# ucla-mobility/QuantV2X

Hardware: AMD Instinct MI355X
Metric: frames/sec/node (N-agent int8 BEV fusion) (higher is better)
Workload: dtype i8

## Files before the change

### include/qv2x.h

```cpp
#ifndef QV2X_H
#define QV2X_H

#include <stdint.h>

#ifdef __cplusplus
extern "C" {
#endif
#if defined(__GNUC__) || defined(__clang__)
#pragma GCC visibility push(default)
#endif

#define QV2X_OK 0
#define QV2X_EINVAL (-1)
#define QV2X_EALIGN (-2)
#define QV2X_MAX_GROUPS 4

const char* qv2x_last_error(void);
#define QV2X_ABI_VERSION 9
int qv2x_version(void);

int qv2x_fill_i8(int8_t* buf, int64_t bytes, int value, void* stream);

int64_t qv2x_voxelize_workspace_bytes(int n_points);
int qv2x_voxelize_f32(const float* points, int n_points, const float* lidar_range, const float* voxel_size, int agent,
// ... 57 lines not shown
                   int8_t* out, void* stream);

int qv2x_deconv_i8_batch(const qv2x_deconv_desc* descs , int n, const int8_t* const* ins ,
                         const float* const* ws, const float* const* biases, int8_t* const* outs, void* stream);

typedef struct {
    int32_t n, h, w;
    int32_t levels, kc;
    int32_t in_zx;
    float in_delta;
    int32_t segs;
} qv2x_encode_desc;
int64_t qv2x_codebook_level_floats(int kc);
int qv2x_codebook_c2_f32(const float* codebook, int kc, float* c2, void* stream);
int qv2x_codebook_encode_f32(const qv2x_encode_desc* desc , const int8_t* in,
                             const float* const* level_weights ,
                             uint8_t* codes, void* stream);
int qv2x_codebook_encode_wave_f32(const qv2x_encode_desc* desc , const int8_t* in, const float* in_f32,
                                  const float* const* level_weights , uint8_t* codes, void* stream);

int qv2x_codebook_encode_collapsed_f32(const qv2x_encode_desc* desc , const int8_t* in, const float* g_packed, const float* bias,
                                       const float* tables, uint8_t* codes, void* stream);

int qv2x_codebook_encode_candidates_i8(const qv2x_encode_desc* desc , const int8_t* in, const int8_t* g_limbs, const double* bias_packed,
                                       const int32_t* tables, const float* tau , uint8_t* codes, uint32_t* list, uint32_t* counters,
                                       void* stream);
int qv2x_codebook_encode_listed_f32(const qv2x_encode_desc* desc , const int8_t* in, const float* const* level_weights ,
                                    const uint32_t* list, const uint32_t* list_count, uint8_t* codes, void* stream);

int qv2x_codebook_encode_candidates_seg_i8(const qv2x_encode_desc* desc , const int8_t* in, const int8_t* g_limbs, const double* bias_packed,
                                           const int32_t* tables, const float* tau , uint8_t* codes, uint32_t* list, uint32_t* counters,
                                           void* stream);

typedef struct {
    int32_t agents, h, w, levels, kc;
    int32_t max_cav, ego;
    int64_t code_agent_stride, code_level_stride;
    double h_metres, w_metres, discrete_ratio;
    int32_t fusion;
} qv2x_fuse_desc;
int qv2x_fuse_att_f32(const qv2x_fuse_desc* desc , const uint8_t* codes, const float* lut, const float* lut_bias,
                      const float* feats, const double* pairwise, float* fused, void* stream);

int qv2x_fuse_att_batch_f32(const qv2x_fuse_desc* desc , int n_scenes, const int64_t* scene_offset ,
                            const int32_t* scene_agents , const uint8_t* codes, const float* lut, const float* lut_bias,
                            const float* feats, const double* pairwise, float* fused, void* stream);

int qv2x_decode_lut_f32(const uint8_t* codes, int R, int levels, int kc, const float* lut, const float* lut_bias,
                        float* out, void* stream);

int qv2x_dequant_i8_f32(const int8_t* in, int n, int h, int w, int c, int zp, float delta, float* out, void* stream);
// ... 188 lines not shown
```

### quantv2x_amd/csrc/codebook_encode.h

```cpp
#pragma once
#include "common.h"

namespace qv2x {

constexpr int ENC_D = 256;
constexpr int ENC_WAVE_PAD = 16 * 256;

struct EncArgs {
    const int8_t* in; const float* in_f32; uint8_t* codes;
    const float* lvl[4];
    int n, h, w, levels, kc, ax, M;
    int segs, ke;
    float dx;
    int m_lo, m_hi;
    int list_slots = 1, list_tail_max = 0;
    const unsigned* list = nullptr; const unsigned* list_count = nullptr;
};

__device__ __host__ __forceinline__ int64_t level_floats_wg(int kc) { return 3LL * (ENC_D * ENC_D + ENC_D) + (int64_t)ENC_D * kc + (int64_t)kc * ENC_D + kc; }
__device__ __host__ __forceinline__ int64_t level_floats(int kc) { return level_floats_wg(kc) + 3LL * ENC_D * ENC_D + (int64_t)((kc + 63) / 64 * 64) * ENC_D + ENC_WAVE_PAD; }

struct ListPlan { int n[3], first[3], total, full; };
__device__ __forceinline__ ListPlan list_plan(const EncArgs& a) {
    ListPlan p;
    int t = 0;
#pragma unroll
    for (int c = 0; c < 3; ++c) { p.n[c] = (int)a.list_count[1 + c]; p.first[c] = t; t += (p.n[c] + 31) >> 5; }
    p.total = t;
    const int full = t / a.list_slots * a.list_slots;
    p.full = t - full > a.list_tail_max ? t : full;
    return p;
}
__device__ __forceinline__ void list_tile(const ListPlan& p, int tile, int& cls, int& i0) {
    cls = tile >= p.first[2] ? 2 : (tile >= p.first[1] ? 1 : 0);
    i0 = (tile - p.first[cls]) * 32;
}

int encode_wave_launch(const EncArgs& a, hipStream_t st);
int encode_wave_list_launch(const EncArgs& a, int waves, hipStream_t st);

}
```

### quantv2x_amd/csrc/codebook_encode.hip

```cpp
#include <cstdlib>

#include <atomic>

#include "codebook_encode.h"

namespace qv2x {

#ifdef QV2X_ENC_TRACE
__device__ unsigned long long g_enc_blk[4096][4];
#endif
#ifdef QV2X_ENC_FINE
__device__ long long g_enc_fine[2048][40];
#define EFINE(k) do { if (threadIdx.x == 0 && blockIdx.x < 2048) g_enc_fine[blockIdx.x][12 * l + (k)] = __builtin_amdgcn_s_memtime(); } while (0)
#else
#define EFINE(k) do { } while (0)
#endif

constexpr int LDF = 258;
__device__ __forceinline__ int kpos(int c) { return (c & ~3) | ((c & 1) << 1) | ((c >> 1) & 1); }
constexpr int D = 256;
#ifndef QV2X_ENC_LDS_PAD
#define QV2X_ENC_LDS_PAD 0
#endif

// ... 304 lines not shown
                for (int r = 0; r < 16; ++r) bufA[(i * 32 + mfma32_row(r, lane)) * LDF + kpos(col)] = acc[i][r] - cv[i][r];
            lds_barrier();
            EFINE(11);
        }
    }
#ifdef QV2X_ENC_TRACE
    if (tid == 0 && blockIdx.x < 4096) {
        g_enc_blk[blockIdx.x][0] = t_start; g_enc_blk[blockIdx.x][1] = __builtin_readcyclecounter();
        g_enc_blk[blockIdx.x][2] = hwid; g_enc_blk[blockIdx.x][3] = xcc;
    }
#endif
}

template <int ER, bool EXT = false>
__global__ __launch_bounds__(512, ER == 32 ? 4 : 2) void codebook_encode_kernel(const EncArgs a) {
    __shared__ __attribute__((aligned(16))) float smem[enc_smem_floats<ER>()];
    encode_rows<ER, EXT>(a, a.m_lo + blockIdx.x * ER, smem);
}

template <bool EXT>
__global__ __launch_bounds__(512, 2) void codebook_encode_list_tail_kernel(const EncArgs a) {
    __shared__ __attribute__((aligned(16))) float smem[enc_smem_floats<32>()];
    const ListPlan plan = list_plan(a);
    for (int t = plan.full + (int)blockIdx.x; t < plan.total; t += (int)gridDim.x) {
        int cls, i0;
        list_tile(plan, t, cls, i0);
        encode_rows<32, EXT, true>(a, i0, smem, a.list + (size_t)cls * a.M, plan.n[cls], cls);
        __syncthreads();
    }
}

template <bool EXT>
__global__ __launch_bounds__(512, 2) void codebook_encode_mixed_kernel(const EncArgs a, const int n64) {
    __shared__ __attribute__((aligned(16))) float smem[enc_smem_floats<64>()];
    if ((int)blockIdx.x < n64) encode_rows<64, EXT>(a, a.m_lo + blockIdx.x * 64, smem);
    else encode_rows<32, EXT>(a, a.m_lo + n64 * 64 + ((int)blockIdx.x - n64) * 32, smem);
}

__global__ void codebook_c2_kernel(const float* __restrict__ cb, int kc, float* __restrict__ c2) {
    const int k = blockIdx.x * blockDim.x + threadIdx.x;
    if (k >= kc) return;
    float s[4];
    for (int q = 0; q < 4; ++q) {
        float acc = 0.0f;
        for (int i = 0; i < 64; ++i) { const float v = cb[(size_t)k * D + q * 64 + i]; acc = fmaf(v, v, acc); }
        s[q] = acc;
    }
// ... 11 lines not shown

extern "C" int64_t qv2x_codebook_level_floats(int kc) { return qv2x::level_floats(kc); }

static int encode_launch(const qv2x_encode_desc* d, const int8_t* in, const float* in_f32, const float* const* level_weights, uint8_t* codes, void* stream,
                         int form = 0);

extern "C" int qv2x_codebook_encode_wave_f32(const qv2x_encode_desc* d, const int8_t* in, const float* in_f32, const float* const* level_weights,
                                             uint8_t* codes, void* stream) {
    if (!in && !in_f32) return qv2x::fail(QV2X_EINVAL, "qv2x_codebook_encode_wave_f32: null pointer");
    return encode_launch(d, in_f32 ? (const int8_t*)in_f32 : in, in_f32, level_weights, codes, stream, 1);
}

extern "C" int qv2x_codebook_encode_f32(const qv2x_encode_desc* d, const int8_t* in, const float* const* level_weights,
                                        uint8_t* codes, void* stream) {
    return encode_launch(d, in, nullptr, level_weights, codes, stream);
}

extern "C" int qv2x_codebook_encode_f32in(const qv2x_encode_desc* d, const float* in, const float* const* level_weights,
                                          uint8_t* codes, void* stream) {
    if (!in) return qv2x::fail(QV2X_EINVAL, "qv2x_codebook_encode_f32in: null pointer");
    return encode_launch(d, (const int8_t*)in, in, level_weights, codes, stream);
}

extern "C" int qv2x_codebook_encode_listed_f32(const qv2x_encode_desc* d, const int8_t* in, const float* const* level_weights,
                                               const uint32_t* list, const uint32_t* list_count, uint8_t* codes, void* stream) {
    using namespace qv2x;
    if (!d || !in || !level_weights || !codes || !list || !list_count) return fail(QV2X_EINVAL, "qv2x_codebook_encode_listed_f32: null pointer");
    if (d->n <= 0 || d->h <= 0 || d->w <= 0 || d->levels < 1 || d->levels > 4) return fail(QV2X_EINVAL, "qv2x_codebook_encode_listed_f32: bad shape");
    const int segs = d->segs ? d->segs : 1;
    if (segs != 1 && segs != 2) return fail(QV2X_EINVAL, "qv2x_codebook_encode_listed_f32: seg_num 1 or 2 (got %d)", d->segs);
    if (d->kc < 32 || d->kc > 256 || d->kc % 32 || (segs > 1 && d->kc % 64) || segs * d->kc > 32 * ENC_MAX_TILES)
        return fail(QV2X_EINVAL, "qv2x_codebook_encode_listed_f32: dict_size must be a multiple of 32 up to 256 (of 64 with two segments): got %d x %d", segs, d->kc);
    if ((uintptr_t)in & 15) return fail(QV2X_EALIGN, "qv2x_codebook_encode_listed_f32: in must be 16-byte aligned");
    EncArgs a;
    a.in = in; a.in_f32 = nullptr; a.codes = codes; a.n = d->n; a.h = d->h; a.w = d->w; a.levels = d->levels; a.kc = d->kc;
    a.segs = segs; a.ke = segs * d->kc;
    const bool ext = segs > 1 || a.ke > 128;
    a.ax = 128 - d->in_zx; a.dx = d->in_delta; a.M = d->n * d->h * d->w; a.m_lo = 0; a.m_hi = a.M;
    a.list = list; a.list_count = list_count;
    for (int l = 0; l < 4; ++l) {
        a.lvl[l] = l < d->levels ? level_weights[l] : nullptr;
        if (l < d->levels && (!a.lvl[l] || ((uintptr_t)a.lvl[l] & 15))) return fail(QV2X_EALIGN, "qv2x_codebook_encode_listed_f32: level %d weights null or unaligned", l);
    }
    int cus = 256, dev = 0, v = 0;
    if (hipGetDevice(&dev) == hipSuccess && hipDeviceGetAttribute(&v, hipDeviceAttributeMultiprocessorCount, dev) == hipSuccess && v > 0) cus = v;
    const int tiles = (a.M + 31) / 32;
    int tail_knob = 0;
#ifdef QV2X_DEV_KNOBS
    static const int tail_env = getenv("QV2X_LIST_TAIL") ? atoi(getenv("QV2X_LIST_TAIL")) : 0;
    tail_knob = tail_env;
#endif
    a.list_slots = 4 * cus; a.list_tail_max = tail_knob > 0 ? tail_knob : 2 * cus;
    const int grid_tail = 2 * cus;
    if (tiles + 3 >= 2 * a.list_slots) {
        if (int rc = encode_wave_list_launch(a, a.list_slots, (hipStream_t)stream)) return rc;
    } else {
        a.list_slots = 1 << 30; a.list_tail_max = 1 << 30;
    }
    if (ext) codebook_encode_list_tail_kernel<true><<<tiles < grid_tail ? tiles : grid_tail, 512, 0, (hipStream_t)stream>>>(a);
    else codebook_encode_list_tail_kernel<false><<<tiles < grid_tail ? tiles : grid_tail, 512, 0, (hipStream_t)stream>>>(a);
    return hip_check(hipGetLastError(), "qv2x_codebook_encode_listed_f32 launch");
}

static int encode_launch(const qv2x_encode_desc* d, const int8_t* in, const float* in_f32, const float* const* level_weights, uint8_t* codes, void* stream,
                         int form) {
    using namespace qv2x;
    if (!d || !in || !level_weights || !codes) return fail(QV2X_EINVAL, "qv2x_codebook_encode_f32: null pointer");
    if (d->n <= 0 || d->h <= 0 || d->w <= 0 || d->levels < 1 || d->levels > 4) return fail(QV2X_EINVAL, "qv2x_codebook_encode_f32: bad shape");
    const int segs = d->segs ? d->segs : 1;
    if (segs != 1 && segs != 2 && segs != 4) return fail(QV2X_EINVAL, "qv2x_codebook_encode_f32: seg_num must be 1, 2 or 4 (got %d)", d->segs);
    if (d->kc < 32 || d->kc > 256 || d->kc % 32 || (segs > 1 && d->kc % 64) || segs * d->kc > 32 * ENC_MAX_TILES)
        return fail(QV2X_EINVAL, "qv2x_codebook_encode_f32: dict_size must be a multiple of 32 up to 256 (of 64 with seg_num > 1; seg_num * dict_size <= %d): "
                                 "got dict_size %d, seg_num %d", 32 * ENC_MAX_TILES, d->kc, segs);
    if ((uintptr_t)in & 15) return fail(QV2X_EALIGN, "qv2x_codebook_encode_f32: in must be 16-byte aligned");
    EncArgs a;
    a.in = in; a.in_f32 = in_f32; a.codes = codes; a.n = d->n; a.h = d->h; a.w = d->w; a.levels = d->levels; a.kc = d->kc;
    a.segs = segs; a.ke = segs * d->kc;
    const bool ext = segs > 1 || a.ke > 128;
    a.ax = 128 - d->in_zx; a.dx = d->in_delta; a.M = d->n * d->h * d->w; a.m_lo = 0; a.m_hi = a.M;
    for (int l = 0; l < 4; ++l) {
        a.lvl[l] = l < d->levels ? level_weights[l] : nullptr;
// ... 63 lines not shown
```

### quantv2x_amd/csrc/codebook_encode_cand.hip

```cpp
#include "common.h"

namespace qv2x {
namespace {

struct CandArgs {
    const int8_t* in; const int8_t* gpack; const double* bias; const int* tables;
    uint8_t* codes; unsigned* list; unsigned* counters;
    float tau[3][3];
    int n, h, w, hw, M, levels, kc, ke, zx, gbytes, tbytes;
    float delta;
};

constexpr int NPF = 8;
constexpr int LIMBS = 3;
template <int V> struct IC { static constexpr int value = V; };

__device__ __forceinline__ double shfl_xor_f64(double v, int m) {
    const long long b = __builtin_bit_cast(long long, v);
    const int lo = __shfl_xor((int)b, m), hi = __shfl_xor((int)(b >> 32), m);
    return __builtin_bit_cast(double, ((long long)hi << 32) | (unsigned)lo);
}

template <int CT, int SEGS, int PACK>
__global__ __launch_bounds__(256) __attribute__((amdgpu_waves_per_eu(1, 1))) void encode_candidates_kernel(const CandArgs a) {
// ... 151 lines not shown
        const unsigned tot = wcnt[0][threadIdx.x] + wcnt[1][threadIdx.x] + wcnt[2][threadIdx.x] + wcnt[3][threadIdx.x];
        wbase[threadIdx.x] = tot ? atomicAdd(a.counters + 1 + threadIdx.x, tot) : 0u;
        if (tot) atomicAdd(a.counters, tot);
    }
    __syncthreads();
    unsigned base[3];
#pragma unroll
    for (int c = 0; c < 3; ++c) {
        base[c] = wbase[c];
        for (int w2 = 0; w2 < wave; ++w2) base[c] += wcnt[w2][c];
    }
#pragma unroll
    for (int c = 0; c < 3; ++c) {
        unsigned at = __builtin_amdgcn_readfirstlane(base[c]);
#pragma unroll
        for (int ct = 0; ct < CT; ++ct) {
            if (first[ct] == c && hf == 0 && m[ct] < a.M)
                a.list[(size_t)c * a.M + at + (unsigned)__builtin_popcountll(mask[c][ct] & ((1ull << lane) - 1ull))] = (unsigned)m[ct];
            at += (unsigned)__builtin_popcountll(mask[c][ct]);
        }
    }
}

__global__ void zero_counters_kernel(unsigned* c) { if (threadIdx.x < 4) c[threadIdx.x] = 0; }

template <int CT, int SEGS, int PACK>
void launch(const CandArgs& a, hipStream_t st) {
    encode_candidates_kernel<CT, SEGS, PACK><<<(a.M + 128 * CT - 1) / (128 * CT), 256, 0, st>>>(a);
}

template <int PACK, int MAX_SEGS>
int candidates(const char* me, const qv2x_encode_desc* d, const int8_t* in, const int8_t* g_limbs, const double* bias_packed, const int32_t* tables,
               const float* tau, uint8_t* codes, uint32_t* list, uint32_t* counters, void* stream) {
    if (!d || !in || !g_limbs || !bias_packed || !tau || !codes || !list || !counters) return fail(QV2X_EINVAL, "%s: null pointer", me);
    if (d->n <= 0 || d->h <= 0 || d->w <= 0 || d->levels < 1 || d->levels > 3) return fail(QV2X_EINVAL, "%s: 1..3 levels", me);
    const int segs = d->segs ? d->segs : 1;
    if (segs < 1 || segs > MAX_SEGS) return fail(QV2X_EINVAL, "%s: seg_num 1 .. %d (got %d; the exact entry takes seg_num 1 | 2 | 4)", me, MAX_SEGS, d->segs);
    if (d->kc < 32 || d->kc > PACK || d->kc % 32 || (segs > 1 && d->kc % 64))
        return fail(QV2X_EINVAL, "%s: dict_size a multiple of 32 up to %d (of 64 with two segments; got %d x %d)", me, PACK, segs, d->kc);
    if (d->levels > 1 && !tables) return fail(QV2X_EINVAL, "%s: the residual levels need their tables", me);
    if (d->in_zx < 0 || d->in_zx > 255) return fail(QV2X_EINVAL, "%s: in_zx outside 0..255", me);
    if (((uintptr_t)in & 15) || ((uintptr_t)g_limbs & 15) || ((uintptr_t)tables & 15) || ((uintptr_t)bias_packed & 7))
        return fail(QV2X_EALIGN, "%s: 16-byte aligned maps, limbs and tables", me);
    CandArgs a;
    a.in = in; a.gpack = g_limbs; a.bias = bias_packed; a.tables = tables; a.codes = codes; a.list = list; a.counters = counters;
    for (int l = 0; l < 3; ++l)
        for (int i = 0; i < 3; ++i) a.tau[l][i] = l < d->levels ? tau[l * 3 + i] : 0.0f;
// ... 29 lines not shown
```

### quantv2x_amd/csrc/codebook_encode_wave.hip

```cpp
#include "codebook_encode.h"

namespace qv2x {

namespace {

constexpr int D = ENC_D;
constexpr int RS = 260;
constexpr int NPF = 4;

__device__ __forceinline__ v16f mfma(float a, float b, v16f c) { return __builtin_amdgcn_mfma_f32_32x32x2f32(a, b, c, 0, 0, 0); }


__device__ __forceinline__ void tile_to_lds(float* __restrict__ row, int h, int T, const v16f& acc) {
#pragma unroll
    for (int rq = 0; rq < 4; ++rq) {
        float* g = row + (4 * T + rq) * 8 + 2 * h;
        *(float2*)g = make_float2(acc[4 * rq], acc[4 * rq + 2]);
        *(float2*)(g + 4) = make_float2(acc[4 * rq + 1], acc[4 * rq + 3]);
    }
}

__device__ __forceinline__ void lds_to_operand(const float* __restrict__ row, int h, float (&m)[128]) {
#pragma unroll
    for (int g = 0; g < 32; ++g) {
// ... 9 lines not shown

#ifdef QV2X_ENCW_FINE
__device__ long long g_encw_fine[4096][32];
#define WFINE(k) do { if (threadIdx.x == 0 && blockIdx.x < 4096) g_encw_fine[blockIdx.x][8 * l + (k)] = __builtin_readcyclecounter(); } while (0)
#define WFINE2(k) do { if (fine2 && threadIdx.x == 0 && blockIdx.x < 4096) g_encw_fine[blockIdx.x][24 + (k)] = __builtin_readcyclecounter(); } while (0)
#define WFINE2_ARM(v) fine2 = (v)
#else
#define WFINE(k) do { } while (0)
#define WFINE2(k) do { } while (0)
#define WFINE2_ARM(v) do { } while (0)
#endif

}

template <int V> struct IC { static constexpr int value = V; };

template <bool F32IN, int SEGS, bool LIST = false>
__global__ __attribute__((amdgpu_flat_work_group_size(64, 64), amdgpu_waves_per_eu(1, 1))) void codebook_encode_wave_kernel(const EncArgs a) {
    __shared__ __attribute__((aligned(16))) float smem[32 * RS];
    const int lane = threadIdx.x, j = lane & 31, h = lane >> 5;
    float* const row = smem + j * RS;
    ListPlan plan{};
    if (LIST) plan = list_plan(a);
#pragma unroll 1
    for (int round = 0; LIST ? round * (int)gridDim.x < plan.full : round == 0; ++round) {
    const int tile = LIST ? round * (int)gridDim.x + ((round & 1) ? (int)gridDim.x - 1 - (int)blockIdx.x : (int)blockIdx.x) : (int)blockIdx.x;
    if (LIST && tile >= plan.full) continue;
    int mrow;
    bool owned;
    int start = 0;
    if (LIST) {
        int cls, i0;
        list_tile(plan, tile, cls, i0);
        owned = i0 + j < plan.n[cls];
        mrow = (int)a.list[(size_t)cls * a.M + (owned ? i0 + j : plan.n[cls] - 1)];
        start = cls;
    } else {
        mrow = a.m_lo + tile * 32 + j;
        owned = mrow < a.m_hi;
    }

    float xq[128], z[128];
    {
        int m = mrow;
        m = m < a.M ? m : a.M - 1;
        const int img = m / (a.h * a.w), rem = m - img * (a.h * a.w);
        const int y = rem / a.w, x = rem - y * a.w;
        const size_t pixel = (size_t)(img * (a.h + 2) + y + 1) * (a.w + 2) + x + 1;
        if (F32IN) {
            const v4f* sf = (const v4f*)(a.in_f32 + pixel * D);
#pragma unroll
            for (int q = 0; q < 64; ++q) {
                const v4f v = sf[q];
                xq[2 * q] = h ? v.y : v.x;
                xq[2 * q + 1] = h ? v.w : v.z;
            }
        } else {
            const v4i* src = (const v4i*)(a.in + pixel * D);
            const float fax = (float)(a.ax - 128);
#pragma unroll
            for (int c = 0; c < 16; ++c) {
                const v4i raw = src[c];
#pragma unroll
                for (int d = 0; d < 4; ++d) {
                    const unsigned u = ((unsigned)raw[d] ^ 0x80808080u) >> (8 * h);
                    xq[8 * c + 2 * d] = ((float)(u & 0xffu) + fax) * a.dx;
                    xq[8 * c + 2 * d + 1] = ((float)((u >> 16) & 0xffu) + fax) * a.dx;
                }
            }
        }
    }

    for (int l = 0; l < a.levels; ++l) {
        const float* W = a.lvl[l];
        const float* stage_b = W + D * D;
        const float* qhead_b = stage_b + D + D * D;
        const float* lhead_b = qhead_b + D + D * D;
        const float* cb = lhead_b + D + (size_t)D * a.ke;
        const float* c2 = cb + (size_t)a.ke * D;
        const __amdgpu_buffer_rsrc_t wrs = __builtin_amdgcn_make_buffer_rsrc((void*)(W + level_floats_wg(a.ke)), 0, 0x7fffffff, 0x00020000);
        int wo = 0;
        const int loff = lane * 16;
        auto wload = [&](int grp) __attribute__((always_inline)) {
            return __builtin_bit_cast(v4f, __builtin_amdgcn_raw_buffer_load_b128(wrs, loff, wo + grp * 1024, 0));
        };
        const bool last = l + 1 == a.levels;
        const int npair = (a.ke + 63) >> 6;

        v4f bn[2][4];
        auto next_vec = [&](const float* p, int P) __attribute__((always_inline)) {
            tile_vec(p, h, 2 * P, bn[0]);
            tile_vec(p, h, 2 * P + 1, bn[1]);
        };
        auto next_c2 = [&](int P) __attribute__((always_inline)) {
            tile_vec(c2, h, 2 * P, bn[0]);
            if (64 * P + 32 < a.ke) tile_vec(c2, h, 2 * P + 1, bn[1]);
// ... 196 lines not shown
        }
        WFINE(5);
        if (last) break;
#pragma unroll 1
        for (int P = 0; P < 4; ++P) {
            const int seg = (P * a.segs) >> 2;
            const float* cw = cb + (size_t)(seg * a.kc + (int)((bcs >> (8 * seg)) & 0xffu)) * D;
            v4f cv[2][4];
            tile_vec(cw, h, 2 * P, cv[0]);
            tile_vec(cw, h, 2 * P + 1, cv[1]);
            __builtin_amdgcn_sched_barrier(0);
            tile2(z, true, [&]() __attribute__((always_inline)) { if (P < 3) next_vec(lhead_b, P + 1); });
#pragma unroll
            for (int t = 0; t < 2; ++t) {
#pragma unroll
                for (int r = 0; r < 16; ++r) acc[t][r] = acc[t][r] - cv[t][r >> 2][r & 3];
                tile_to_lds(row, h, 2 * P + t, acc[t]);
            }
        }
        WFINE(6);
        lds_to_operand(row, h, xq);
        WFINE(7);
    }
    }
}

int encode_wave_launch(const EncArgs& a, hipStream_t st) {
    const unsigned grid = (unsigned)((a.m_hi - a.m_lo + 31) / 32);
    if (a.segs == 2) {
        if (a.in_f32) codebook_encode_wave_kernel<true, 2><<<grid, 64, 0, st>>>(a);
        else codebook_encode_wave_kernel<false, 2><<<grid, 64, 0, st>>>(a);
    } else if (a.segs == 4) {
        if (a.in_f32) codebook_encode_wave_kernel<true, 4><<<grid, 64, 0, st>>>(a);
        else codebook_encode_wave_kernel<false, 4><<<grid, 64, 0, st>>>(a);
    } else if (a.in_f32) codebook_encode_wave_kernel<true, 1><<<grid, 64, 0, st>>>(a);
    else codebook_encode_wave_kernel<false, 1><<<grid, 64, 0, st>>>(a);
    return hip_check(hipGetLastError(), "qv2x_codebook_encode_f32 (wave form) launch");
}


int encode_wave_list_launch(const EncArgs& a, int waves, hipStream_t st) {
    if ((a.segs != 1 && a.segs != 2) || a.in_f32) return fail(QV2X_EINVAL, "qv2x_codebook_encode_listed_f32: seg_num 1 | 2, i8 rows");
    if (a.segs == 2) codebook_encode_wave_kernel<false, 2, true><<<(unsigned)waves, 64, 0, st>>>(a);
    else codebook_encode_wave_kernel<false, 1, true><<<(unsigned)waves, 64, 0, st>>>(a);
    return hip_check(hipGetLastError(), "qv2x_codebook_encode_listed_f32 launch");
}
// ... 9 lines not shown
```

### quantv2x_amd/engine.py

```python
from __future__ import annotations

import ctypes as C
from typing import Dict, List, Optional

import numpy as np
import torch
import torch.nn as nn

from . import lib as L
from .ptq_state import export_ptq_state, load_ptq_state

_HEADS = ("cls_head", "reg_head", "dir_head")


def _dev(a: np.ndarray, dev) -> torch.Tensor:
    return torch.from_numpy(np.ascontiguousarray(a)).to(dev).contiguous()


def _pack_k4(w: np.ndarray) -> np.ndarray:
    j, k = w.shape
    assert k % 4 == 0
    return np.ascontiguousarray(w.T.reshape(k // 4, 4, j).transpose(0, 2, 1), dtype=np.float32)


# ... 438 lines not shown
        (_, h0, w0) = b["lvl"][0]
        self.fh, self.fw = h0 * self.ups[0], w0 * self.ups[0]
        for lvl, (_, hl, wl) in enumerate(b["lvl"]):
            if (hl * self.ups[lvl], wl * self.ups[lvl]) != (self.fh, self.fw):
                raise ValueError(f"deblock {lvl} upsamples {hl}x{wl} by {self.ups[lvl]} to {hl * self.ups[lvl]}x{wl * self.ups[lvl]}, "
                                 f"level 0 gives {self.fh}x{self.fw}: the grid does not line up across backbone levels")
        cat = torch.empty((n, self.fh + 2, self.fw + 2, self.cat_channels), dtype=torch.int8, device=self.dev)
        c0 = 0
        for de in self.deblocks:
            cat[..., c0:c0 + de.cout] = int(de.out_q[1]) - 128
            c0 += de.cout
        b["cat"] = cat
        b["s0"] = self._padded(n, self.fh, self.fw, self.shrink0.cout, self.shrink0.out_q)
        b["s1"] = self._padded(n, self.fh, self.fw, self.shrink1.cout, self.shrink1.out_q)
        if self.compress:
            b["comp"] = [self._padded(n, self.fh, self.fw, c.cout, c.out_q) for c in self.comp]
        hw = self.fh * self.fw
        if self.has_codebook:
            b["codes"] = torch.empty((self.levels, n, hw), dtype=torch.uint8, device=self.dev)
        if self.two_stage_supported():
            if self._two_stage is None and self.encode_mode == "two_stage":
                self._build_two_stage()
            b["enc_list"] = torch.zeros(3 * n * hw, dtype=torch.int32, device=self.dev)
            b["enc_counters"] = torch.zeros(4, dtype=torch.int32, device=self.dev)
        if not self.has_codebook or self.heads_single is not None:
            b["feats"] = torch.empty((n, hw, 256), dtype=torch.float32, device=self.dev)
        self._bufs[n] = b
        return b

    def _conv(self, layer: _ConvLayer, x, n, h, w, out, out_ctotal=None, out_c0=0):
        d = L.ConvDesc()
        d.n, d.h, d.w, d.cin_total, d.stride, d.cout = n, h, w, x.shape[-1], layer.stride, layer.cout
        d.ngroups = len(layer.groups)
        for i, (c0, c, zx) in enumerate(layer.groups):
            d.group_c0[i], d.group_c[i], d.group_zx[i] = c0, c, zx
        d.out_ctotal = out.shape[-1] if out_ctotal is None else out_ctotal
        d.out_c0, d.relu = out_c0, 1
        d.out_delta, d.out_zp = layer.out_q[0], float(layer.out_q[1])
        if self.use_wide_conv and self.lib.qv2x_conv3x3_i8_wide_ok(C.byref(d)):
            if layer.w_wide is None:
                layer.w_wide = torch.empty_like(layer.w)
                L.check(self.lib.qv2x_conv3x3_i8_pack_wide(C.byref(d), L.ptr(layer.w), L.ptr(layer.w_wide), L.current_stream()), layer.name)
            L.check(self.lib.qv2x_conv3x3_i8_wide(C.byref(d), L.ptr(x), L.ptr(layer.w_wide), L.ptr(layer.scale), L.ptr(layer.corr),
                                                  L.ptr(layer.aw), L.ptr(layer.bias), L.ptr(out), L.current_stream()), layer.name)
            return
        L.check(self.lib.qv2x_conv3x3_i8(C.byref(d), L.ptr(x), L.ptr(layer.w), L.ptr(layer.scale), L.ptr(layer.corr),
                                         L.ptr(layer.aw), L.ptr(layer.bias), L.ptr(out), L.current_stream()), layer.name)
# ... 598 lines not shown
```

### quantv2x_amd/lib.py

```python
from __future__ import annotations

import ctypes as C
import os

_HERE = os.path.dirname(os.path.abspath(__file__))
LIB_PATH = os.path.join(_HERE, "libqv2x.so")
MAX_GROUPS = 4
ABI_VERSION = 9

SYMBOLS = [
    "qv2x_last_error", "qv2x_version", "qv2x_fill_i8", "qv2x_pfn_scatter_i8", "qv2x_pfn_unscatter_i8", "qv2x_conv3x3_i8",
    "qv2x_conv3x3_i8_wide_ok", "qv2x_conv3x3_i8_pack_wide", "qv2x_conv3x3_i8_wide", "qv2x_conv3x3_i8_chain64",
    "qv2x_deconv_i8", "qv2x_deconv_i8_batch", "qv2x_codebook_level_floats", "qv2x_codebook_c2_f32", "qv2x_codebook_encode_f32", "qv2x_codebook_encode_wave_f32", "qv2x_fuse_att_f32", "qv2x_fuse_att_batch_f32", "qv2x_fuse_heads_batch_f32",
    "qv2x_decode_lut_f32", "qv2x_single_heads_lut_f32", "qv2x_table_heads_f32", "qv2x_dequant_i8_f32", "qv2x_heads_f32", "qv2x_decode_heads_f32", "qv2x_heads_pair_f32", "qv2x_voxelize_workspace_bytes", "qv2x_voxelize_f32",
    "qv2x_postprocess_workspace_bytes", "qv2x_postprocess_f32", "qv2x_postprocess_late_workspace_bytes", "qv2x_postprocess_late_f32",
    "qv2x_conv3x3_f32", "qv2x_deconv_f32", "qv2x_pfn_scatter_f32", "qv2x_codebook_encode_f32in",
    "qv2x_pyramid_weighted_fuse_f32", "qv2x_pyramid_weighted_fuse_i8", "qv2x_conv1x1_i8", "qv2x_gconv3x3_i8", "qv2x_conv3x3_i8_res",
    "qv2x_deconv_f32in", "qv2x_codebook_decode_f32", "qv2x_occ_score_i8",
    "qv2x_codebook64_level_floats", "qv2x_codebook64_c2_f32", "qv2x_codebook_encode64_f32", "qv2x_codebook_encode64_f32in",
    "qv2x_add_relu_f32", "qv2x_occ_sigmoid_f32", "qv2x_pyramid_weighted_fuse_f32p", "qv2x_bottleneck_i8",
    "qv2x_comm_unique_id", "qv2x_comm_init", "qv2x_comm_destroy", "qv2x_allgather_codes", "qv2x_pairwise_from_poses_f64", "qv2x_pairwise_from_poses_batch_f64",
    "qv2x_codebook_encode_collapsed_f32", "qv2x_codebook_encode_candidates_i8", "qv2x_codebook_encode_candidates_seg_i8", "qv2x_codebook_encode_listed_f32", "qv2x_mean_vfe_f32", "qv2x_sp_index_scatter", "qv2x_sp_out_sites_workspace_bytes", "qv2x_sp_out_sites", "qv2x_sp_rulebook", "qv2x_sp_conv_f32in", "qv2x_sp_conv_i8", "qv2x_sp_to_bev_i8",
    "qv2x_fuse_att_band_f32", "qv2x_heads_band", "qv2x_fuse_heads_band", "qv2x_assemble_bands",
    "qv2x_voxelize_batch_workspace_bytes", "qv2x_voxelize_batch_f32", "qv2x_postprocess_batch_workspace_bytes", "qv2x_postprocess_batch_f32",
]
WIRES = {"f32": 0, "u8": 1}
COMM_ID_BYTES = 128


class PfnParams(C.Structure):
    _fields_ = [("w", C.c_float * 640), ("b", C.c_float * 64),
                ("d1", C.c_float), ("z1", C.c_float), ("d2", C.c_float), ("z2", C.c_float),
                ("vox", C.c_float * 3), ("off", C.c_float * 3)]


class ConvDesc(C.Structure):
    _fields_ = [("n", C.c_int32), ("h", C.c_int32), ("w", C.c_int32), ("cin_total", C.c_int32),
                ("stride", C.c_int32), ("cout", C.c_int32), ("ngroups", C.c_int32),
                ("group_c0", C.c_int32 * MAX_GROUPS), ("group_c", C.c_int32 * MAX_GROUPS),
                ("group_zx", C.c_int32 * MAX_GROUPS),
                ("out_ctotal", C.c_int32), ("out_c0", C.c_int32), ("relu", C.c_int32),
                ("out_delta", C.c_float), ("out_zp", C.c_float)]


class ChainDesc(C.Structure):
# ... 96 lines not shown
    lib.qv2x_deconv_i8.argtypes = [C.POINTER(DeconvDesc), vp, vp, vp, vp, vp]
    lib.qv2x_deconv_i8_batch.argtypes = [C.POINTER(DeconvDesc), C.c_int, C.POINTER(vp), C.POINTER(vp), C.POINTER(vp), C.POINTER(vp), vp]
    lib.qv2x_codebook_level_floats.argtypes = [C.c_int]
    lib.qv2x_codebook_level_floats.restype = C.c_int64
    lib.qv2x_codebook_c2_f32.argtypes = [vp, C.c_int, vp, vp]
    lib.qv2x_codebook_encode_f32.argtypes = [C.POINTER(EncodeDesc), vp, C.POINTER(vp), vp, vp]
    lib.qv2x_codebook_encode_wave_f32.argtypes = [C.POINTER(EncodeDesc), vp, vp, C.POINTER(vp), vp, vp]
    lib.qv2x_fuse_att_f32.argtypes = [C.POINTER(FuseDesc), vp, vp, vp, vp, vp, vp, vp]
    lib.qv2x_fuse_att_batch_f32.argtypes = [C.POINTER(FuseDesc), C.c_int, C.POINTER(C.c_int64), C.POINTER(C.c_int32), vp, vp, vp, vp, vp, vp, vp]
    lib.qv2x_decode_lut_f32.argtypes = [vp, C.c_int, C.c_int, C.c_int, vp, vp, vp, vp]
    lib.qv2x_fuse_heads_batch_f32.argtypes = [C.POINTER(FuseDesc), C.c_int, C.POINTER(C.c_int64), C.POINTER(C.c_int32), vp, vp, vp, vp, vp,
                                              C.c_int, C.c_int, vp, vp, vp, vp, vp, vp, vp]
    lib.qv2x_heads_f32.argtypes = [vp, C.c_int, C.c_int, C.c_int, C.c_int, vp, vp, vp, vp, vp, vp]
    lib.qv2x_decode_heads_f32.argtypes = [vp, C.c_int, C.c_int, C.c_int, C.c_int, vp, vp, C.c_int, C.c_int, vp, vp, vp, vp, vp, vp]
    lib.qv2x_table_heads_f32.argtypes = [vp, C.c_int, C.c_int, C.c_int, C.c_int, C.c_int, C.c_int, vp, vp, vp, vp, vp, vp, vp]
    lib.qv2x_single_heads_lut_f32.argtypes = [vp, C.c_int, C.c_int, C.c_int, C.c_int, C.c_int, vp, vp, vp, vp, vp, vp]
    lib.qv2x_heads_pair_f32.argtypes = [vp, C.c_int, C.c_int, C.c_int, C.c_int, vp, vp, vp, vp, vp,
                                        vp, C.c_int, C.c_int, C.c_int, vp, vp, C.c_int, C.c_int, vp, vp, vp, vp, vp, vp]
    lib.qv2x_dequant_i8_f32.argtypes = [vp, C.c_int, C.c_int, C.c_int, C.c_int, C.c_int, C.c_float, vp, vp]
    lib.qv2x_codebook_encode_collapsed_f32.argtypes = [C.POINTER(EncodeDesc), vp, vp, vp, vp, vp, vp]
    lib.qv2x_codebook_encode_candidates_i8.argtypes = [C.POINTER(EncodeDesc), vp, vp, vp, vp, C.POINTER(C.c_float), vp, vp, vp, vp]
    lib.qv2x_codebook_encode_candidates_seg_i8.argtypes = [C.POINTER(EncodeDesc), vp, vp, vp, vp, C.POINTER(C.c_float), vp, vp, vp, vp]
    lib.qv2x_codebook_encode_listed_f32.argtypes = [C.POINTER(EncodeDesc), vp, C.POINTER(vp), vp, vp, vp, vp]
    lib.qv2x_mean_vfe_f32.argtypes = [vp, vp, vp, C.c_int, C.c_int, vp, vp]
    lib.qv2x_sp_index_scatter.argtypes = [vp, vp, C.c_int, C.c_int, C.c_int, C.c_int, C.c_int, vp, C.c_int, vp]
    lib.qv2x_sp_out_sites_workspace_bytes.argtypes = [C.POINTER(SpconvDesc)]
    lib.qv2x_sp_out_sites_workspace_bytes.restype = C.c_int64
    lib.qv2x_sp_out_sites.argtypes = [C.POINTER(SpconvDesc), vp, vp, vp, vp, vp, vp, C.c_int64, vp]
    lib.qv2x_sp_rulebook.argtypes = [C.POINTER(SpconvDesc), vp, vp, vp, vp, vp]
    lib.qv2x_sp_conv_f32in.argtypes = [C.POINTER(SpconvDesc), vp, vp, vp, vp, vp, vp, vp, vp]
    lib.qv2x_sp_conv_i8.argtypes = [C.POINTER(SpconvDesc), vp, vp, vp, vp, vp, vp, vp, vp, vp, vp, vp]
    lib.qv2x_sp_to_bev_i8.argtypes = [vp, vp, vp, C.c_int, C.c_int, C.c_int, C.c_int, C.c_int, C.c_int, C.c_int, C.c_int, vp, vp]
    lib.qv2x_voxelize_workspace_bytes.argtypes = [C.c_int]
    lib.qv2x_voxelize_workspace_bytes.restype = C.c_int64
    lib.qv2x_voxelize_f32.argtypes = [vp, C.c_int, C.POINTER(C.c_float), C.POINTER(C.c_float), C.c_int, C.c_int, C.c_int,
                                      vp, C.c_int64, vp, vp, vp, vp, vp]
    lib.qv2x_voxelize_batch_workspace_bytes.argtypes = [C.c_int, C.POINTER(C.c_int32)]
    lib.qv2x_voxelize_batch_workspace_bytes.restype = C.c_int64
    lib.qv2x_voxelize_batch_f32.argtypes = [C.POINTER(vp), C.POINTER(C.c_int32), C.c_int, C.POINTER(C.c_float), C.POINTER(C.c_float),
                                            C.c_int, C.c_int, C.c_int, vp, C.c_int64, vp, vp, vp, vp, vp]
    lib.qv2x_postprocess_batch_workspace_bytes.argtypes = [C.POINTER(PostprocessDesc), C.c_int]
    lib.qv2x_postprocess_batch_workspace_bytes.restype = C.c_int64
    lib.qv2x_postprocess_batch_f32.argtypes = [C.POINTER(PostprocessDesc), C.c_int, vp, C.c_int64, vp, C.c_int64, vp, C.c_int64, vp, vp,
                                               vp, C.c_int64, vp, vp, vp, vp, vp]
    lib.qv2x_postprocess_workspace_bytes.argtypes = [C.POINTER(PostprocessDesc)]
    lib.qv2x_postprocess_workspace_bytes.restype = C.c_int64
# ... 66 lines not shown
```

Before: 6912.

## Replace static round-robin list tiles with atomic work queue in wave encode

The listed encode wave kernel stops assigning tiles in fixed round-robin rounds. Each workgroup now takes its next tile from a global atomic ticket counter, drawn during the last level so the fetch overlaps compute, and the last workgroup to finish resets the counter. The split between the wave kernel and the workgroup tail kernel moves from a fixed tail size to a share derived from a modeled ratio. A host-side plan/predict API is added to expose this split. The aim is better load balance across classes of uneven cost, at the cost of atomics and a counter buffer widened to 8 entries that callers must pass.

```diff
diff --git a/include/qv2x.h b/include/qv2x.h
--- a/include/qv2x.h
+++ b/include/qv2x.h
@@ -103,11 +103,14 @@
 int qv2x_codebook_encode_collapsed_f32(const qv2x_encode_desc* desc , const int8_t* in, const float* g_packed, const float* bias,
                                        const float* tables, uint8_t* codes, void* stream);
 
+#define QV2X_ENCODE_COUNTERS 8
 int qv2x_codebook_encode_candidates_i8(const qv2x_encode_desc* desc , const int8_t* in, const int8_t* g_limbs, const double* bias_packed,
                                        const int32_t* tables, const float* tau , uint8_t* codes, uint32_t* list, uint32_t* counters,
                                        void* stream);
 int qv2x_codebook_encode_listed_f32(const qv2x_encode_desc* desc , const int8_t* in, const float* const* level_weights ,
-                                    const uint32_t* list, const uint32_t* list_count, uint8_t* codes, void* stream);
+                                    const uint32_t* list, uint32_t* counters, uint8_t* codes, void* stream);
+int qv2x_codebook_encode_list_plan(const qv2x_encode_desc* desc , int cus, const uint32_t* counts , int32_t* out ,
+                                   double* predicted , int32_t* weights , double* rho );
 
 int qv2x_codebook_encode_candidates_seg_i8(const qv2x_encode_desc* desc , const int8_t* in, const int8_t* g_limbs, const double* bias_packed,
                                            const int32_t* tables, const float* tau , uint8_t* codes, uint32_t* list, uint32_t* counters,
diff --git a/quantv2x_amd/csrc/codebook_encode.h b/quantv2x_amd/csrc/codebook_encode.h
--- a/quantv2x_amd/csrc/codebook_encode.h
+++ b/quantv2x_amd/csrc/codebook_encode.h
@@ -13,25 +13,37 @@
     int segs, ke;
     float dx;
     int m_lo, m_hi;
-    int list_slots = 1, list_tail_max = 0;
+    int list_slots = 1, list_wg_max = 0;
     const unsigned* list = nullptr; const unsigned* list_count = nullptr;
+    unsigned* list_queue = nullptr;
 };
 
 __device__ __host__ __forceinline__ int64_t level_floats_wg(int kc) { return 3LL * (ENC_D * ENC_D + ENC_D) + (int64_t)ENC_D * kc + (int64_t)kc * ENC_D + kc; }
 __device__ __host__ __forceinline__ int64_t level_floats(int kc) { return level_floats_wg(kc) + 3LL * ENC_D * ENC_D + (int64_t)((kc + 63) / 64 * 64) * ENC_D + ENC_WAVE_PAD; }
 
-struct ListPlan { int n[3], first[3], total, full; };
-__device__ __forceinline__ ListPlan list_plan(const EncArgs& a) {
+constexpr int LIST_RHO_PCT = 59;
+__host__ __device__ constexpr int list_wg_rounds() { return 100 / LIST_RHO_PCT; }
+__host__ __device__ constexpr int list_wg_share(int grid) { return list_wg_rounds() * grid; }
+static_assert(LIST_RHO_PCT >= 1 && LIST_RHO_PCT <= 100, "a round of workgroups that outlasts a wave tile: the workgroup form has no share");
+
+__host__ __device__ __forceinline__ int list_cut(int total, int slots, int wg_max) {
+    if (total <= wg_max) return 0;
+    const long long rounds = ((long long)total - wg_max + slots - 1) / slots;
+    return rounds * slots > total ? total : (int)(rounds * slots);
+}
+
+struct ListPlan { int n[3], first[3], total, cut; };
+__host__ __device__ __forceinline__ ListPlan list_plan_of(const unsigned* counts, int slots, int wg_max) {
     ListPlan p;
     int t = 0;
 #pragma unroll
-    for (int c = 0; c < 3; ++c) { p.n[c] = (int)a.list_count[1 + c]; p.first[c] = t; t += (p.n[c] + 31) >> 5; }
+    for (int c = 0; c < 3; ++c) { p.n[c] = (int)counts[c]; p.first[c] = t; t += (p.n[c] + 31) >> 5; }
     p.total = t;
-    const int full = t / a.list_slots * a.list_slots;
-    p.full = t - full > a.list_tail_max ? t : full;
+    p.cut = list_cut(t, slots, wg_max);
     return p;
 }
-__device__ __forceinline__ void list_tile(const ListPlan& p, int tile, int& cls, int& i0) {
+__device__ __forceinline__ ListPlan list_plan(const EncArgs& a) { return list_plan_of(a.list_count + 1, a.list_slots, a.list_wg_max); }
+__host__ __device__ __forceinline__ void list_tile(const ListPlan& p, int tile, int& cls, int& i0) {
     cls = tile >= p.first[2] ? 2 : (tile >= p.first[1] ? 1 : 0);
     i0 = (tile - p.first[cls]) * 32;
 }
diff --git a/quantv2x_amd/csrc/codebook_encode.hip b/quantv2x_amd/csrc/codebook_encode.hip
--- a/quantv2x_amd/csrc/codebook_encode.hip
+++ b/quantv2x_amd/csrc/codebook_encode.hip
@@ -350,7 +350,7 @@
 __global__ __launch_bounds__(512, 2) void codebook_encode_list_tail_kernel(const EncArgs a) {
     __shared__ __attribute__((aligned(16))) float smem[enc_smem_floats<32>()];
     const ListPlan plan = list_plan(a);
-    for (int t = plan.full + (int)blockIdx.x; t < plan.total; t += (int)gridDim.x) {
+    for (int t = plan.cut + (int)blockIdx.x; t < plan.total; t += (int)gridDim.x) {
         int cls, i0;
         list_tile(plan, t, cls, i0);
         encode_rows<32, EXT, true>(a, i0, smem, a.list + (size_t)cls * a.M, plan.n[cls], cls);
@@ -408,10 +408,78 @@
     return encode_launch(d, (const int8_t*)in, in, level_weights, codes, stream);
 }
 
+namespace qv2x {
+namespace {
+
+struct ListShape { int tiles, slots, grid, wg_max; bool waves; };
+ListShape list_shape(int m_cells, int cus) {
+    ListShape s;
+    s.tiles = (m_cells + 31) / 32; s.slots = 4 * cus; s.grid = 2 * cus;
+    s.waves = s.tiles + 3 >= 2 * s.slots;
+    s.wg_max = list_wg_share(s.grid);
+    if (!s.waves) { s.slots = 1 << 30; s.wg_max = 1 << 30; }
+    return s;
+}
+
+void list_weights(int levels, int kc, int segs, int (&w)[3]) {
+    const int dist = segs == 1 ? (kc + 63) / 64 : kc / 64;
+    for (int c = 0; c < 3; ++c) {
+        w[c] = 0;
+        for (int l = 0; l < levels; ++l) w[c] += 4 + (l >= c ? 4 + dist : 0) + (l + 1 < levels ? 4 : 0);
+    }
+}
+
+double list_predict(const ListPlan& p, const ListShape& s, const int (&w)[3]) {
+    auto prefix = [&](int t) {
+        double c = 0;
+        for (int k = 0; k < 3; ++k) {
+            const int end = k < 2 ? p.first[k + 1] : p.total;
+            const int n = (t < end ? t : end) - p.first[k];
+            if (n > 0) c += (double)n * w[k];
+        }
+        return c;
+    };
+    const int whole = p.cut / s.slots * s.slots, ragged = p.cut - whole;
+    double t = prefix(whole) / s.slots;
+    if (ragged) t += (prefix(p.cut) - prefix(whole)) / ragged;
+    for (int r = p.cut; r < p.total; r += s.grid) {
+        int cls, i0;
+        list_tile(p, r, cls, i0);
+        t += LIST_RHO_PCT / 100.0 * w[cls];
+    }
+    return t;
+}
+
+}
+}
+
+extern "C" int qv2x_codebook_encode_list_plan(const qv2x_encode_desc* d, int cus, const uint32_t* counts, int32_t* out, double* predicted,
+                                              int32_t* weights, double* rho) {
+    using namespace qv2x;
+    if (!d || !counts || !out || cus <= 0) return fail(QV2X_EINVAL, "qv2x_codebook_encode_list_plan: null pointer or no compute units");
+    if (d->n <= 0 || d->h <= 0 || d->w <= 0 || d->levels < 1 || d->levels > 4) return fail(QV2X_EINVAL, "qv2x_codebook_encode_list_plan: bad shape");
+    const int m_cells = d->n * d->h * d->w;
+    for (int c = 0; c < 3; ++c)
+        if (counts[c] > (uint32_t)m_cells) return fail(QV2X_EINVAL, "qv2x_codebook_encode_list_plan: list %d longer than the map", c);
+    const ListShape s = list_shape(m_cells, cus);
+    const ListPlan p = list_plan_of(counts, s.slots, s.wg_max);
+    int w[3];
+    list_weights(d->levels, d->kc, d->segs ? d->segs : 1, w);
+    out[0] = p.total; out[1] = p.cut; out[2] = s.waves ? s.slots : 0; out[3] = s.grid;
+    if (predicted) {
+        ListShape ps = s;
+        if (!s.waves) ps.slots = 1;
+        *predicted = list_predict(p, ps, w);
+    }
+    if (weights) for (int c = 0; c < 3; ++c) weights[c] = w[c];
+    if (rho) *rho = LIST_RHO_PCT / 100.0;
+    return QV2X_OK;
+}
+
 extern "C" int qv2x_codebook_encode_listed_f32(const qv2x_encode_desc* d, const int8_t* in, const float* const* level_weights,
-                                               const uint32_t* list, const uint32_t* list_count, uint8_t* codes, void* stream) {
+                                               const uint32_t* list, uint32_t* counters, uint8_t* codes, void* stream) {
     using namespace qv2x;
-    if (!d || !in || !level_weights || !codes || !list || !list_count) return fail(QV2X_EINVAL, "qv2x_codebook_encode_listed_f32: null pointer");
+    if (!d || !in || !level_weights || !codes || !list || !counters) return fail(QV2X_EINVAL, "qv2x_codebook_encode_listed_f32: null pointer");
     if (d->n <= 0 || d->h <= 0 || d->w <= 0 || d->levels < 1 || d->levels > 4) return fail(QV2X_EINVAL, "qv2x_codebook_encode_listed_f32: bad shape");
     const int segs = d->segs ? d->segs : 1;
     if (segs != 1 && segs != 2) return fail(QV2X_EINVAL, "qv2x_codebook_encode_listed_f32: seg_num 1 or 2 (got %d)", d->segs);
@@ -423,26 +491,23 @@
     a.segs = segs; a.ke = segs * d->kc;
     const bool ext = segs > 1 || a.ke > 128;
     a.ax = 128 - d->in_zx; a.dx = d->in_delta; a.M = d->n * d->h * d->w; a.m_lo = 0; a.m_hi = a.M;
-    a.list = list; a.list_count = list_count;
+    a.list = list; a.list_count = counters;
     for (int l = 0; l < 4; ++l) {
         a.lvl[l] = l < d->levels ? level_weights[l] : nullptr;
         if (l < d->levels && (!a.lvl[l] || ((uintptr_t)a.lvl[l] & 15))) return fail(QV2X_EALIGN, "qv2x_codebook_encode_listed_f32: level %d weights null or unaligned", l);
     }
+    a.list_queue = counters + 4;
     int cus = 256, dev = 0, v = 0;
     if (hipGetDevice(&dev) == hipSuccess && hipDeviceGetAttribute(&v, hipDeviceAttributeMultiprocessorCount, dev) == hipSuccess && v > 0) cus = v;
-    const int tiles = (a.M + 31) / 32;
-    int tail_knob = 0;
+    const ListShape shape = list_shape(a.M, cus);
+    a.list_slots = shape.slots; a.list_wg_max = shape.wg_max;
 #ifdef QV2X_DEV_KNOBS
-    static const int tail_env = getenv("QV2X_LIST_TAIL") ? atoi(getenv("QV2X_LIST_TAIL")) : 0;
-    tail_knob = tail_env;
-#endif
-    a.list_slots = 4 * cus; a.list_tail_max = tail_knob > 0 ? tail_knob : 2 * cus;
-    const int grid_tail = 2 * cus;
-    if (tiles + 3 >= 2 * a.list_slots) {
+    static const char* const share_env = getenv("QV2X_LIST_WG_MAX");
+    if (share_env && shape.waves) a.list_wg_max = atoi(share_env);
+#endif
+    const int tiles = shape.tiles, grid_tail = shape.grid;
+    if (shape.waves)
         if (int rc = encode_wave_list_launch(a, a.list_slots, (hipStream_t)stream)) return rc;
-    } else {
-        a.list_slots = 1 << 30; a.list_tail_max = 1 << 30;
-    }
     if (ext) codebook_encode_list_tail_kernel<true><<<tiles < grid_tail ? tiles : grid_tail, 512, 0, (hipStream_t)stream>>>(a);
     else codebook_encode_list_tail_kernel<false><<<tiles < grid_tail ? tiles : grid_tail, 512, 0, (hipStream_t)stream>>>(a);
     return hip_check(hipGetLastError(), "qv2x_codebook_encode_listed_f32 launch");
diff --git a/quantv2x_amd/csrc/codebook_encode_cand.hip b/quantv2x_amd/csrc/codebook_encode_cand.hip
--- a/quantv2x_amd/csrc/codebook_encode_cand.hip
+++ b/quantv2x_amd/csrc/codebook_encode_cand.hip
@@ -197,7 +197,7 @@
     }
 }
 
-__global__ void zero_counters_kernel(unsigned* c) { if (threadIdx.x < 4) c[threadIdx.x] = 0; }
+__global__ void zero_counters_kernel(unsigned* c) { if (threadIdx.x < QV2X_ENCODE_COUNTERS) c[threadIdx.x] = 0; }
 
 template <int CT, int SEGS, int PACK>
 void launch(const CandArgs& a, hipStream_t st) {
diff --git a/quantv2x_amd/csrc/codebook_encode_wave.hip b/quantv2x_amd/csrc/codebook_encode_wave.hip
--- a/quantv2x_amd/csrc/codebook_encode_wave.hip
+++ b/quantv2x_amd/csrc/codebook_encode_wave.hip
@@ -55,10 +55,15 @@
     float* const row = smem + j * RS;
     ListPlan plan{};
     if (LIST) plan = list_plan(a);
-#pragma unroll 1
-    for (int round = 0; LIST ? round * (int)gridDim.x < plan.full : round == 0; ++round) {
-    const int tile = LIST ? round * (int)gridDim.x + ((round & 1) ? (int)gridDim.x - 1 - (int)blockIdx.x : (int)blockIdx.x) : (int)blockIdx.x;
-    if (LIST && tile >= plan.full) continue;
+    const int late = LIST && plan.cut >= (int)gridDim.x ? plan.cut % (int)gridDim.x : 0, early = (int)gridDim.x - late;
+    const int queue_end = plan.cut - late;
+    int tile = (int)blockIdx.x < early ? (int)blockIdx.x : plan.cut - 1 - ((int)blockIdx.x - early);
+    bool first_tile = true;
+#pragma unroll 1
+    for (;;) {
+    if (LIST && (first_tile ? tile >= plan.cut : tile >= queue_end)) break;
+    first_tile = false;
+    unsigned ticket = 0;
     int mrow;
     bool owned;
     int start = 0;
@@ -105,6 +110,7 @@
     }
 
     for (int l = 0; l < a.levels; ++l) {
+        if (LIST && l + 1 == a.levels && lane == 0) ticket = __hip_atomic_fetch_add(a.list_queue, 1u, __ATOMIC_RELAXED, __HIP_MEMORY_SCOPE_AGENT);
         const float* W = a.lvl[l];
         const float* stage_b = W + D * D;
         const float* qhead_b = stage_b + D + D * D;
@@ -347,6 +353,12 @@
         lds_to_operand(row, h, xq);
         WFINE(7);
     }
+    if (!LIST) break;
+    tile = early + (int)__builtin_amdgcn_readfirstlane(ticket);
+    }
+    if (LIST && lane == 0 && __hip_atomic_fetch_add(a.list_queue + 1, 1u, __ATOMIC_RELAXED, __HIP_MEMORY_SCOPE_AGENT) == gridDim.x - 1) {
+        __hip_atomic_store(a.list_queue, 0u, __ATOMIC_RELAXED, __HIP_MEMORY_SCOPE_AGENT);
+        __hip_atomic_store(a.list_queue + 1, 0u, __ATOMIC_RELAXED, __HIP_MEMORY_SCOPE_AGENT);
     }
 }
 
diff --git a/quantv2x_amd/engine.py b/quantv2x_amd/engine.py
--- a/quantv2x_amd/engine.py
+++ b/quantv2x_amd/engine.py
@@ -484,7 +484,8 @@
             if self._two_stage is None and self.encode_mode == "two_stage":
                 self._build_two_stage()
             b["enc_list"] = torch.zeros(3 * n * hw, dtype=torch.int32, device=self.dev)
-            b["enc_counters"] = torch.zeros(4, dtype=torch.int32, device=self.dev)
+            b["enc_counters_all"] = torch.zeros(8, dtype=torch.int32, device=self.dev)
+            b["enc_counters"] = b["enc_counters_all"][:4]
         if not self.has_codebook or self.heads_single is not None:
             b["feats"] = torch.empty((n, hw, 256), dtype=torch.float32, device=self.dev)
         self._bufs[n] = b
diff --git a/quantv2x_amd/lib.py b/quantv2x_amd/lib.py
--- a/quantv2x_amd/lib.py
+++ b/quantv2x_amd/lib.py
@@ -20,7 +20,7 @@
     "qv2x_codebook64_level_floats", "qv2x_codebook64_c2_f32", "qv2x_codebook_encode64_f32", "qv2x_codebook_encode64_f32in",
     "qv2x_add_relu_f32", "qv2x_occ_sigmoid_f32", "qv2x_pyramid_weighted_fuse_f32p", "qv2x_bottleneck_i8",
     "qv2x_comm_unique_id", "qv2x_comm_init", "qv2x_comm_destroy", "qv2x_allgather_codes", "qv2x_pairwise_from_poses_f64", "qv2x_pairwise_from_poses_batch_f64",
-    "qv2x_codebook_encode_collapsed_f32", "qv2x_codebook_encode_candidates_i8", "qv2x_codebook_encode_candidates_seg_i8", "qv2x_codebook_encode_listed_f32", "qv2x_mean_vfe_f32", "qv2x_sp_index_scatter", "qv2x_sp_out_sites_workspace_bytes", "qv2x_sp_out_sites", "qv2x_sp_rulebook", "qv2x_sp_conv_f32in", "qv2x_sp_conv_i8", "qv2x_sp_to_bev_i8",
+    "qv2x_codebook_encode_collapsed_f32", "qv2x_codebook_encode_candidates_i8", "qv2x_codebook_encode_candidates_seg_i8", "qv2x_codebook_encode_listed_f32", "qv2x_codebook_encode_list_plan", "qv2x_mean_vfe_f32", "qv2x_sp_index_scatter", "qv2x_sp_out_sites_workspace_bytes", "qv2x_sp_out_sites", "qv2x_sp_rulebook", "qv2x_sp_conv_f32in", "qv2x_sp_conv_i8", "qv2x_sp_to_bev_i8",
     "qv2x_fuse_att_band_f32", "qv2x_heads_band", "qv2x_fuse_heads_band", "qv2x_assemble_bands",
     "qv2x_voxelize_batch_workspace_bytes", "qv2x_voxelize_batch_f32", "qv2x_postprocess_batch_workspace_bytes", "qv2x_postprocess_batch_f32",
 ]
@@ -163,6 +163,8 @@
     lib.qv2x_codebook_encode_candidates_i8.argtypes = [C.POINTER(EncodeDesc), vp, vp, vp, vp, C.POINTER(C.c_float), vp, vp, vp, vp]
     lib.qv2x_codebook_encode_candidates_seg_i8.argtypes = [C.POINTER(EncodeDesc), vp, vp, vp, vp, C.POINTER(C.c_float), vp, vp, vp, vp]
     lib.qv2x_codebook_encode_listed_f32.argtypes = [C.POINTER(EncodeDesc), vp, C.POINTER(vp), vp, vp, vp, vp]
+    lib.qv2x_codebook_encode_list_plan.argtypes = [C.POINTER(EncodeDesc), C.c_int, C.POINTER(C.c_uint32), C.POINTER(C.c_int32), C.POINTER(C.c_double),
+                                                   C.POINTER(C.c_int32), C.POINTER(C.c_double)]
     lib.qv2x_mean_vfe_f32.argtypes = [vp, vp, vp, C.c_int, C.c_int, vp, vp]
     lib.qv2x_sp_index_scatter.argtypes = [vp, vp, C.c_int, C.c_int, C.c_int, C.c_int, C.c_int, vp, C.c_int, vp]
     lib.qv2x_sp_out_sites_workspace_bytes.argtypes = [C.POINTER(SpconvDesc)]
```

Result: no change. 6902 (-0.1%).
